# qc-tum/TNC

Measured on NVIDIA H100. Metric: pairwise contractions/sec (effective ZGEMM TFLOP/s in zgemm_tflops), higher is better.
Workload: dtype f64

## Files before the change

### include/tncb.h

```cpp
#ifndef TNCB_H
#define TNCB_H

#include <stddef.h>
#include <stdint.h>

#ifdef __cplusplus
extern "C" {
#endif

typedef enum tncb_status {
  TNCB_OK = 0,
  TNCB_ERR_INVALID = -1,
  TNCB_ERR_SHAPE = -2,
  TNCB_ERR_UNCONTRACTED = -3,
  TNCB_ERR_NOT_CONTRACTED = -4,
  TNCB_ERR_OOM = -5,
  TNCB_ERR_CUDA = -6,
  TNCB_ERR_GATE = -7,
  TNCB_ERR_NCCL = -8,
  TNCB_ERR_UNSUPPORTED = -9,
  TNCB_ERR_IO = -10
} tncb_status;

typedef struct tncb_ctx tncb_ctx;
// ... 8 lines not shown
int tncb_ctx_create(int device, size_t arena_bytes, tncb_ctx** out);
void tncb_ctx_destroy(tncb_ctx* ctx);
int tncb_ctx_synchronize(tncb_ctx* ctx);
void* tncb_ctx_stream(tncb_ctx* ctx);
int tncb_ctx_trim(tncb_ctx* ctx, uint64_t* freed_bytes, uint64_t* reserved_bytes);
int tncb_ctx_stats(tncb_ctx* ctx, uint64_t* kernel_launches, uint64_t* arena_peak_bytes,
                   uint64_t* arena_live_bytes);
int tncb_ctx_reset_stats(tncb_ctx* ctx);
int tncb_ctx_set_tcgen05_slices(tncb_ctx* ctx, int slices);
int tncb_ctx_set_tcgen05_engine(tncb_ctx* ctx, int engine);
int tncb_ctx_set_tolerance(tncb_ctx* ctx, double rel);
int tncb_ctx_set_tcgen05_moduli(tncb_ctx* ctx, int n_moduli);
int tncb_ctx_set_tcgen05_products(tncb_ctx* ctx, int products, long long min_k3);
int tncb_tcgen05_bound(uint64_t k, double rel, int n_moduli_force, int* n_moduli, int* bits_a, int* bits_b, double* bound);
int tncb_tcgen05_tables(int n_moduli, int* moduli, double* rho1, double* rho2, double* log2_product);
int tncb_ctx_set_tcgen05_workspace(tncb_ctx* ctx, size_t bytes);
int tncb_ctx_set_tcgen05_threshold(tncb_ctx* ctx, long long min_tiles, long long min_k);
int tncb_ctx_engine_counts(tncb_ctx* ctx, uint64_t counts[8]);
int tncb_ctx_last_tcgen05_info(tncb_ctx* ctx, double* int8_ops, int* n_moduli);
int tncb_ctx_last_tcgen05_products(tncb_ctx* ctx, int* products);
int tncb_ctx_time_gemm(tncb_ctx* ctx, int enable);
int tncb_ctx_last_gemm_ms(tncb_ctx* ctx, float* ms);
int tncb_ctx_gemm_totals(tncb_ctx* ctx, double* ms, double* int8_ops, uint64_t* launches);

int tncb_tensor_upload(tncb_ctx* ctx, int rank, const uint64_t* dims,
                       const double* host_re_im, tncb_tensor** out);
int tncb_tensor_alloc(tncb_ctx* ctx, int rank, const uint64_t* dims, tncb_tensor** out);
int tncb_tensor_download(tncb_ctx* ctx, const tncb_tensor* t, double* host_re_im);
int tncb_tensor_write(tncb_ctx* ctx, tncb_tensor* t, const double* host_re_im);
int tncb_tensor_read(tncb_ctx* ctx, const tncb_tensor* t, double* host_re_im);
int tncb_tensor_free(tncb_ctx* ctx, tncb_tensor* t);
int tncb_tensor_rank(const tncb_tensor* t);
int tncb_tensor_dims(const tncb_tensor* t, uint64_t* dims_out);
uint64_t tncb_tensor_elements(const tncb_tensor* t);
void* tncb_tensor_device_ptr(const tncb_tensor* t);

int tncb_contract_pair(tncb_ctx* ctx, int n_out, const uint64_t* out_legs,
                       int n_a, const uint64_t* a_legs, tncb_tensor* a,
                       int n_b, const uint64_t* b_legs, tncb_tensor* b,
                       tncb_tensor** out);
int tncb_contract_pair_keep(tncb_ctx* ctx, int n_a, const uint64_t* a_legs, const tncb_tensor* a,
                            int n_b, const uint64_t* b_legs, const tncb_tensor* b,
                            tncb_tensor** out);
int tncb_contract_pair_into(tncb_ctx* ctx, int n_a, const uint64_t* a_legs, const tncb_tensor* a,
                            int n_b, const uint64_t* b_legs, const tncb_tensor* b,
                            tncb_tensor* out);
// ... 137 lines not shown
```

### tnc_b200/__init__.py

```python
from __future__ import annotations

import ctypes as C
from typing import Sequence

import numpy as np

from ._lib import TncbError, check, lib, u64_array

__all__ = ["Context", "DeviceTensor", "TncbError", "contract_pair", "contract_pair_into", "default_context", "lib"]


class Context:

    def __init__(self, device: int = 0, arena_bytes: int = 0):
        self._l = lib()
        h = C.c_void_p()
        check(self._l.tncb_ctx_create(device, arena_bytes, C.byref(h)))
        self.handle = h
        self.device = device

    def synchronize(self) -> None:
        check(self._l.tncb_ctx_synchronize(self.handle))

    @property
# ... 31 lines not shown
    def engine_counts(self) -> dict:
        arr = (C.c_uint64 * 8)()
        check(self._l.tncb_ctx_engine_counts(self.handle, arr))
        names = ["k0", "k0_splitk", "k1_dmma", "k1_dmma_splitk", "k1_tcgen05", "k2", "permute", "reserved"]
        return {n: int(arr[i]) for i, n in enumerate(names)}

    def last_tcgen05_info(self) -> dict:
        ops, n = C.c_double(), C.c_int()
        check(self._l.tncb_ctx_last_tcgen05_info(self.handle, C.byref(ops), C.byref(n)))
        pr = C.c_int()
        check(self._l.tncb_ctx_last_tcgen05_products(self.handle, C.byref(pr)))
        return {"int8_ops": ops.value, "n_moduli": n.value, "products": pr.value}

    def set_tcgen05_threshold(self, min_tiles: int, min_k: int) -> None:
        check(self._l.tncb_ctx_set_tcgen05_threshold(self.handle, int(min_tiles), int(min_k)))

    def time_gemm(self, enable=True) -> None:
        check(self._l.tncb_ctx_time_gemm(self.handle, int(enable)))

    def gemm_totals(self) -> dict:
        ms, ops, n = C.c_double(), C.c_double(), C.c_uint64()
        check(self._l.tncb_ctx_gemm_totals(self.handle, C.byref(ms), C.byref(ops), C.byref(n)))
        return {"ms": ms.value, "int8_ops": ops.value, "launches": n.value}

    def last_gemm_ms(self) -> float:
        ms = C.c_float()
        check(self._l.tncb_ctx_last_gemm_ms(self.handle, C.byref(ms)))
        return float(ms.value)

    def reset_stats(self) -> None:
        check(self._l.tncb_ctx_reset_stats(self.handle))

    def close(self) -> None:
        if getattr(self, "handle", None):
            self._l.tncb_ctx_destroy(self.handle)
            self.handle = None

    def __del__(self):
        try:
            self.close()
        except Exception:
            pass


_default_ctx = None

# ... 161 lines not shown
```

### tnc_b200/_lib.py

```python
from __future__ import annotations

import ctypes as C
import os

_HERE = os.path.dirname(os.path.abspath(__file__))
LIB_PATH = os.path.join(_HERE, "lib", "libtncb200.so")

u64p = C.POINTER(C.c_uint64)
f64p = C.POINTER(C.c_double)
i32p = C.POINTER(C.c_int)
vpp = C.POINTER(C.c_void_p)


class TncbTn(C.Structure):
    pass


TncbTn._fields_ = [
    ("n_children", C.c_size_t),
    ("children", C.POINTER(TncbTn)),
    ("rank", C.c_int),
    ("legs", u64p),
    ("dims", u64p),
    ("kind", C.c_int),
# ... 27 lines not shown
    "tncb_ctx_create": (C.c_int, [C.c_int, C.c_size_t, vpp]),
    "tncb_ctx_destroy": (None, [C.c_void_p]),
    "tncb_ctx_synchronize": (C.c_int, [C.c_void_p]),
    "tncb_ctx_stream": (C.c_void_p, [C.c_void_p]),
    "tncb_ctx_stats": (C.c_int, [C.c_void_p, u64p, u64p, u64p]),
    "tncb_ctx_reset_stats": (C.c_int, [C.c_void_p]),
    "tncb_ctx_set_tcgen05_slices": (C.c_int, [C.c_void_p, C.c_int]),
    "tncb_ctx_set_tcgen05_engine": (C.c_int, [C.c_void_p, C.c_int]),
    "tncb_ctx_set_tolerance": (C.c_int, [C.c_void_p, C.c_double]),
    "tncb_ctx_set_tcgen05_moduli": (C.c_int, [C.c_void_p, C.c_int]),
    "tncb_tcgen05_bound": (C.c_int, [C.c_uint64, C.c_double, C.c_int, i32p, i32p, i32p, f64p]),
    "tncb_tcgen05_tables": (C.c_int, [C.c_int, i32p, f64p, f64p, f64p]),
    "tncb_ctx_set_tcgen05_workspace": (C.c_int, [C.c_void_p, C.c_size_t]),
    "tncb_ctx_engine_counts": (C.c_int, [C.c_void_p, u64p]),
    "tncb_ctx_last_tcgen05_info": (C.c_int, [C.c_void_p, f64p, i32p]),
    "tncb_ctx_last_tcgen05_products": (C.c_int, [C.c_void_p, i32p]),
    "tncb_ctx_trim": (C.c_int, [C.c_void_p, u64p, u64p]),
    "tncb_path_reconfigure": (C.c_int, [C.c_int, C.c_int, u64p, f64p, i32p, C.c_int, C.c_int, C.c_double, f64p, C.c_uint64, f64p, f64p, f64p]),
    "tncb_path_leg_scores": (C.c_int, [C.c_int, C.c_int, u64p, f64p, i32p, C.c_double, f64p, f64p, f64p, f64p, f64p]),
    "tncb_ctx_set_tcgen05_products": (C.c_int, [C.c_void_p, C.c_int, C.c_longlong]),
    "tncb_ctx_set_tcgen05_threshold": (C.c_int, [C.c_void_p, C.c_longlong, C.c_longlong]),
    "tncb_ctx_time_gemm": (C.c_int, [C.c_void_p, C.c_int]),
    "tncb_ctx_gemm_totals": (C.c_int, [C.c_void_p, f64p, f64p, u64p]),
    "tncb_ctx_last_gemm_ms": (C.c_int, [C.c_void_p, C.POINTER(C.c_float)]),
    "tncb_tensor_upload": (C.c_int, [C.c_void_p, C.c_int, u64p, C.c_void_p, vpp]),
    "tncb_tensor_alloc": (C.c_int, [C.c_void_p, C.c_int, u64p, vpp]),
    "tncb_tensor_download": (C.c_int, [C.c_void_p, C.c_void_p, C.c_void_p]),
    "tncb_tensor_write": (C.c_int, [C.c_void_p, C.c_void_p, C.c_void_p]),
    "tncb_tensor_read": (C.c_int, [C.c_void_p, C.c_void_p, C.c_void_p]),
    "tncb_tensor_free": (C.c_int, [C.c_void_p, C.c_void_p]),
    "tncb_tensor_rank": (C.c_int, [C.c_void_p]),
    "tncb_tensor_dims": (C.c_int, [C.c_void_p, u64p]),
    "tncb_tensor_elements": (C.c_uint64, [C.c_void_p]),
    "tncb_tensor_device_ptr": (C.c_void_p, [C.c_void_p]),
    "tncb_contract_pair": (C.c_int, [C.c_void_p, C.c_int, u64p, C.c_int, u64p, C.c_void_p, C.c_int, u64p, C.c_void_p, vpp]),
    "tncb_contract_pair_keep": (C.c_int, [C.c_void_p, C.c_int, u64p, C.c_void_p, C.c_int, u64p, C.c_void_p, vpp]),
    "tncb_contract_pair_into": (C.c_int, [C.c_void_p, C.c_int, u64p, C.c_void_p, C.c_int, u64p, C.c_void_p, C.c_void_p]),
    "tncb_contract_pair_host": (C.c_int, [C.c_void_p, C.c_int, u64p, u64p, C.c_void_p, C.c_int, u64p, u64p, C.c_void_p, C.c_void_p]),
    "tncb_pair_out_legs": (C.c_int, [C.c_int, u64p, u64p, C.c_int, u64p, u64p, i32p, u64p, u64p, u64p, u64p, u64p]),
    "tncb_pair_kernel_class": (C.c_int, [C.c_int, u64p, u64p, C.c_int, u64p, u64p]),
    "tncb_permute": (C.c_int, [C.c_void_p, C.c_void_p, i32p, vpp]),
    "tncb_conjugate": (C.c_int, [C.c_void_p, C.c_void_p]),
    "tncb_tensor_add": (C.c_int, [C.c_void_p, C.c_void_p, C.c_void_p]),
    "tncb_gate_matrix": (C.c_int, [C.c_char_p, f64p, C.c_int, C.c_int, f64p, i32p]),
    "tncb_contract_tensor_network": (C.c_int, [C.c_void_p, C.POINTER(TncbTn), C.POINTER(TncbPath), vpp, i32p, u64p]),
    "tncb_network_out_legs": (C.c_int, [C.POINTER(TncbTn), C.POINTER(TncbPath), i32p, u64p, u64p]),
# ... 90 lines not shown
```

### tnc_b200/csrc/crt.cu

```cuda
#include "internal.h"
#include "sm90.h"
#include <cuda.h>
#include <algorithm>
#include <cmath>
#include <cstdio>
#include <cstdlib>

namespace tncb {

constexpr int CRT_MAX_MOD = 20;
static const int kModuli[CRT_MAX_MOD] = {256, 253, 251, 249, 247, 245, 241, 239, 233, 229,
                                         227, 223, 211, 199, 197, 193, 191, 181, 179, 173};
constexpr int CRT_BT = 128;
constexpr int CRT_BKB = WG_BKB;
#ifndef CRT_RING3_STAGES
#define CRT_RING3_STAGES 3
#endif
#ifndef CRT_RING3_BK
#define CRT_RING3_BK 128
#endif
#ifndef CRT_RING4_STAGES
#define CRT_RING4_STAGES 5
#endif
#ifndef CRT_RING4_BK
// ... 126 lines not shown
#pragma unroll
  for (int it = 0; it < RES_ROWS_C * RES_K_C / 256; it++) {
    int r, k;
    crt_tile_coord(it * 256 + tid, lk, r, k);
    unsigned long long m = mv[it];
    for (int d = 1; d < (1 << lk); d <<= 1) m = max(m, __shfl_xor_sync(0xffffffffu, m, d));
    if (r != cur_r) {
      if (cur_m && (tid & ((1 << lk) - 1)) == 0) atomicMax(&s_max[cur_r], cur_m);
      cur_r = r; cur_m = 0ull;
    }
    cur_m = max(cur_m, m);
  }
  if (cur_m && (tid & ((1 << lk) - 1)) == 0) atomicMax(&s_max[cur_r], cur_m);
  __syncthreads();
  if (tid < RES_ROWS_C && row0 + tid < rows && s_max[tid] != 0ull) atomicMax(rowmax + row0 + tid, s_max[tid]);
}

__device__ __forceinline__ int crt_fix_byte(int s, int m) {
  if (s > 127) s -= m;
  else if (s < -128) s += m;
  return s;
}
constexpr int RES_ROWS = RES_ROWS_C, RES_K = RES_K_C, RES_RS = RES_K + RES_K / 8 + 1;
template <int COMPS, bool KARA>
__global__ void __launch_bounds__(256, 3)
crt_residue_kernel(const double2* __restrict__ src, const long long* __restrict__ off_row, const long long* __restrict__ off_k,
                   long long rows, long long K, long long rowsP, long long Kp, const unsigned long long* __restrict__ rowmax, int bits, int lk,
                   const __grid_constant__ CrtTables T, int8_t* __restrict__ planes) {
  extern __shared__ __align__(16) unsigned char res_smem_raw[];
  double2* tile = reinterpret_cast<double2*>(res_smem_raw);
  __shared__ double s_scale[RES_ROWS];
  __shared__ long long s_offr[RES_ROWS], s_offk[RES_K];
  __shared__ double s_inv[CRT_MAX_MOD];
  __shared__ int s_mod[CRT_MAX_MOD];
  const long long row0 = (long long)blockIdx.x * RES_ROWS, k0 = (long long)blockIdx.y * RES_K;
  const int tid = threadIdx.x;
  const double two_a = scalbn(1.0, bits);
  if (tid >= 64 && tid < 64 + CRT_MAX_MOD) { s_inv[tid - 64] = T.inv_mod[tid - 64]; s_mod[tid - 64] = T.mod[tid - 64]; }
  if (tid < RES_ROWS) {
    const long long r = row0 + tid;
    const int e = r < rows ? crt_exp_from_bits(rowmax[r]) : 0;
    s_scale[tid] = (e == kExpNonFinite) ? 0.0 : scalbn(1.0, -e);
    s_offr[tid] = r < rows ? __ldg(off_row + r) : -1;
  } else if (tid >= 128) {
    const int k = tid - 128;
    s_offk[k] = k0 + k < K ? __ldg(off_k + k0 + k) : -1;
  }
  __syncthreads();
  double2 vv[RES_ROWS * RES_K / 256];
#pragma unroll
  for (int it = 0; it < RES_ROWS * RES_K / 256; it++) {
    int r, k;
    crt_tile_coord(it * 256 + tid, lk, r, k);
    const long long orow = s_offr[r], ok = s_offk[k];
    vv[it] = make_double2(0.0, 0.0);
    if (orow >= 0 && ok >= 0) vv[it] = __ldg(src + orow + ok);
  }
#pragma unroll
  for (int it = 0; it < RES_ROWS * RES_K / 256; it++) {
    int r, k;
    crt_tile_coord(it * 256 + tid, lk, r, k);
    const double sc = s_scale[r];
    double2 v = vv[it];
    v.x = trunc(v.x * sc * two_a);
    v.y = trunc(v.y * sc * two_a);
    if (sc == 0.0) { v.x = 0.0; v.y = 0.0; }
    tile[r * RES_RS + k + (k >> 3)] = v;
  }
  __syncthreads();
  const int r = tid >> 3;
  if (row0 + r >= rows) return;
  const double RMAGIC = 6755399441055744.0;
  const long long plane_stride = rowsP * Kp;
#pragma unroll 1
  for (int pass = 0; pass < 2; pass++) {
    const int g = (tid & 7) + 8 * pass;
    double xr[8], xi[8];
    int lr[8], li[8];
#pragma unroll
    for (int j = 0; j < 8; j++) {
      const double2 v = tile[r * RES_RS + g * 9 + j];
      xr[j] = v.x; xi[j] = v.y;
      lr[j] = (int)__double2ll_rn(v.x); li[j] = (int)__double2ll_rn(v.y);
    }
    int8_t* dst = planes + (row0 + r) * Kp + k0 + g * 8;
    const int nmod = T.nmod;
#pragma unroll 1
    for (int i = 0; i < nmod; i++) {
      const int m = s_mod[i];
      const double inv = s_inv[i];
      uint32_t wr[2] = {0, 0}, wi[2] = {0, 0}, ws[2] = {0, 0};
#pragma unroll
      for (int j = 0; j < 8; j++) {
        const int qr = __double2loint(fma(xr[j], inv, RMAGIC));
        const int qi = __double2loint(fma(xi[j], inv, RMAGIC));
        const int rr = lr[j] - qr * m, ri = li[j] - qi * m;
        constexpr uint32_t sel[4] = {0x3214u, 0x3240u, 0x3410u, 0x4210u};
        wr[j >> 2] = __byte_perm(wr[j >> 2], (uint32_t)rr, sel[j & 3]);
        wi[j >> 2] = __byte_perm(wi[j >> 2], (uint32_t)ri, sel[j & 3]);
        if (KARA) ws[j >> 2] = __byte_perm(ws[j >> 2], (uint32_t)crt_fix_byte(rr + ri, m), sel[j & 3]);
      }
      int8_t* d = dst + (long long)i * (KARA ? 3 : COMPS) * plane_stride;
      if (KARA) {
        *reinterpret_cast<uint2*>(d) = make_uint2(wr[0], wr[1]);
        *reinterpret_cast<uint2*>(d + plane_stride) = make_uint2(wi[0], wi[1]);
        *reinterpret_cast<uint2*>(d + 2 * plane_stride) = make_uint2(ws[0], ws[1]);
      } else if (COMPS == 2) {
        *reinterpret_cast<uint2*>(d) = make_uint2(wr[0], wr[1]);
        *reinterpret_cast<uint2*>(d + plane_stride) = make_uint2(wi[0], wi[1]);
// ... 295 lines not shown
    return (size_t)nmod * (size_t)Kp * (size_t)(NPB * n_ + 3 * m_) + (size_t)nmod * nkc * NPR * (size_t)n_ * (size_t)m_;
  };
  while (ws_bytes(pn, pm) > budget && (pm > TM || pn > CRT_BT)) {
    if (pm >= pn && pm > TM) pm = round_up_ll(pm / 2, TM);
    else if (pn > CRT_BT) pn = round_up_ll(pn / 2, CRT_BT);
    else pm = round_up_ll(pm / 2, TM);
  }
  const size_t bytesB = (size_t)nmod * NPB * pn * Kp, bytesA = (size_t)nmod * 3 * pm * Kp;
  const size_t bytesR = (size_t)nmod * nkc * NPR * pn * pm;
  const size_t bytesE = (size_t)(pn + pm) * sizeof(unsigned long long);
  void *pb = nullptr, *pa = nullptr, *pr = nullptr, *pe = nullptr;
  int rc;
  if ((rc = ctx->arena.alloc(bytesB, &pb))) return rc;
  if ((rc = ctx->arena.alloc(bytesA, &pa))) { ctx->arena.free(pb, bytesB); return rc; }
  if ((rc = ctx->arena.alloc(bytesR, &pr))) { ctx->arena.free(pb, bytesB); ctx->arena.free(pa, bytesA); return rc; }
  if ((rc = ctx->arena.alloc(bytesE, &pe))) { ctx->arena.free(pb, bytesB); ctx->arena.free(pa, bytesA); ctx->arena.free(pr, bytesR); return rc; }
  auto cleanup = [&]() { ctx->arena.free(pb, bytesB); ctx->arena.free(pa, bytesA); ctx->arena.free(pr, bytesR); ctx->arena.free(pe, bytesE); };
  unsigned long long* max_n = (unsigned long long*)pe;
  unsigned long long* max_m = max_n + pn;

  static bool attr_done_dev[64] = {false};
  bool& attr_done = attr_done_dev[ctx->device & 63];
  const int smem_gemm4 = CrtRing<false>::SMEM, smem_gemm3 = CrtRing<true>::SMEM;
  const int smem_res = RES_ROWS * RES_RS * (int)sizeof(double2);
  if (!attr_done) {
    cudaError_t e = cudaFuncSetAttribute(crt_gemm_kernel<false>, cudaFuncAttributeMaxDynamicSharedMemorySize, smem_gemm4);
    if (e == cudaSuccess) e = cudaFuncSetAttribute(crt_gemm_kernel<true>, cudaFuncAttributeMaxDynamicSharedMemorySize, smem_gemm3);
    if (e == cudaSuccess) e = cudaFuncSetAttribute(crt_residue_kernel<2, false>, cudaFuncAttributeMaxDynamicSharedMemorySize, smem_res);
    if (e == cudaSuccess) e = cudaFuncSetAttribute(crt_residue_kernel<3, false>, cudaFuncAttributeMaxDynamicSharedMemorySize, smem_res);
    if (e == cudaSuccess) e = cudaFuncSetAttribute(crt_residue_kernel<2, true>, cudaFuncAttributeMaxDynamicSharedMemorySize, smem_res);
    if (e == cudaSuccess) e = cudaFuncSetAttribute(crt_residue_kernel<3, true>, cudaFuncAttributeMaxDynamicSharedMemorySize, smem_res);
    if (e != cudaSuccess) { cleanup(); return fail(TNCB_ERR_CUDA, cudaGetErrorString(e)); }
    attr_done = true;
  }
  auto lane_split = [](const LegList& kl, bool k_is_b, const LegList& fl) {
    auto p2 = [](long long d) { int b = 0; while ((2LL << b) <= d && b < 5) b++; return b; };
    const long long ks = kl.n ? (k_is_b ? kl.sb[kl.n - 1] : kl.sa[kl.n - 1]) : (1LL << 62);
    const long long fs = fl.n ? fl.sa[fl.n - 1] : (1LL << 62);
    if (ks <= fs) return kl.n ? p2(kl.dim[kl.n - 1]) : 0;
    return 0;
  };
  const int lk_b = lane_split(P.k, true, P.n), lk_a = lane_split(P.k, false, P.m);
  ctx->last_int8_ops = 0.0; ctx->last_nmod = nmod; ctx->last_products = kara ? 3 : 4;
  bool timed = false;

  for (long long n0 = 0; n0 < P.N; n0 += pn) {
    const long long nrows = std::min(pn, P.N - n0);
    const long long Np = round_up_ll(nrows, CRT_BT);
    if (Np != nrows) cudaMemsetAsync(pb, 0, (size_t)nmod * NPB * Np * Kp, st);
    cudaMemsetAsync(max_n, 0, (size_t)nrows * sizeof(unsigned long long), st);
    {
      dim3 g((unsigned)((nrows + RES_ROWS - 1) / RES_ROWS), (unsigned)(Kp / RES_K));
      crt_rowmax_kernel<<<g, 256, 0, st>>>(B, offBn + n0, offBk, nrows, P.K, lk_b, max_n);
      if (kara) crt_residue_kernel<2, true><<<g, 256, smem_res, st>>>(B, offBn + n0, offBk, nrows, P.K, Np, Kp, max_n, bits_b, lk_b, T, (int8_t*)pb);
      else crt_residue_kernel<2, false><<<g, 256, smem_res, st>>>(B, offBn + n0, offBk, nrows, P.K, Np, Kp, max_n, bits_b, lk_b, T, (int8_t*)pb);
    }
    ctx->launches += 2;
    CUtensorMap mapB;
    if ((rc = kara ? wg_make_map<CrtRing<true>::BK>(&mapB, pb, (uint64_t)nmod * NPB * Np, (uint64_t)Kp)
                   : wg_make_map<CrtRing<false>::BK>(&mapB, pb, (uint64_t)nmod * NPB * Np, (uint64_t)Kp))) { cleanup(); return rc; }
    for (long long m0 = 0; m0 < P.M; m0 += pm) {
      const long long mcols = std::min(pm, P.M - m0);
      const long long Mp = round_up_ll(mcols, TM);
      if (Mp != mcols) cudaMemsetAsync(pa, 0, (size_t)nmod * 3 * Mp * Kp, st);
      cudaMemsetAsync(max_m, 0, (size_t)mcols * sizeof(unsigned long long), st);
      {
        dim3 g((unsigned)((mcols + RES_ROWS - 1) / RES_ROWS), (unsigned)(Kp / RES_K));
        crt_rowmax_kernel<<<g, 256, 0, st>>>(A, offAm + m0, offAk, mcols, P.K, lk_a, max_m);
        if (kara) crt_residue_kernel<3, true><<<g, 256, smem_res, st>>>(A, offAm + m0, offAk, mcols, P.K, Mp, Kp, max_m, bits_a, lk_a, T, (int8_t*)pa);
        else crt_residue_kernel<3, false><<<g, 256, smem_res, st>>>(A, offAm + m0, offAk, mcols, P.K, Mp, Kp, max_m, bits_a, lk_a, T, (int8_t*)pa);
      }
      ctx->launches += 2;
      CUtensorMap mapA;
      if ((rc = kara ? wg_make_map<CrtRing<true>::BK>(&mapA, pa, (uint64_t)nmod * 3 * Mp, (uint64_t)Kp)
                     : wg_make_map<CrtRing<false>::BK>(&mapA, pa, (uint64_t)nmod * 3 * Mp, (uint64_t)Kp))) { cleanup(); return rc; }
      CrtGemmArgs g;
      g.R = (int8_t*)pr; g.Np = (int)Np; g.Mp = (int)Mp;
      g.tiles_n = (int)(Np / CRT_BT); g.tiles_m = (int)(Mp / TM); g.tile_m = TM;
      g.nmod = nmod; g.nkc = nkc; g.kb_per_chunk = kb_per_chunk; g.num_kb = num_kb;
      const long long items = (long long)g.tiles_n * g.tiles_m * nmod * nkc * (kara ? 3 : 1);
      if (items > 0x7fffffffLL) { cleanup(); return fail(TNCB_ERR_UNSUPPORTED, "too many work items"); }
      g.total_items = (int)items;
      g.group = ctx->crt_group;
      for (int i = 0; i < CRT_MAX_MOD; i++) { g.negmod[i] = -T.mod[i]; g.magic[i] = T.magic[i]; }
      const unsigned grid = (unsigned)std::min<long long>(ctas_max, items);
      const double ops = 2.0 * (kara ? 3.0 : 4.0) * (double)nmod * (double)Np * (double)Mp * (double)Kp;
      const bool time_this = ctx->time_gemm == 2 || (ctx->time_gemm == 1 && !timed);
      if (time_this) gemm_timer_begin(ctx);
      if (kara) crt_gemm_kernel<true><<<grid, WG_THREADS, smem_gemm3, st>>>(mapB, mapA, g);
      else crt_gemm_kernel<false><<<grid, WG_THREADS, smem_gemm4, st>>>(mapB, mapA, g);
      cudaError_t e = cudaGetLastError();
      if (time_this) { gemm_timer_end(ctx, ops); timed = true; }
      if (e != cudaSuccess) { cleanup(); return fail(TNCB_ERR_CUDA, std::string("crt_gemm_kernel launch: ") + cudaGetErrorString(e)); }
      ctx->last_int8_ops += ops;
      CrtReconArgs r;
      r.R = (const int8_t*)pr; r.C = C + n0 * P.M + m0; r.max_n = max_n; r.max_m = max_m;
      r.rows = nrows; r.cols = mcols; r.ldc = P.M; r.Np = Np; r.Mp = Mp; r.nkc = nkc;
      const long long threads = nrows * (Mp / 4);
      const unsigned rg = (unsigned)((threads + 255) / 256);
      if (kara) {
        if (nkc == 1) crt_reconstruct_kernel<true, true><<<rg, 256, 0, st>>>(r, T);
        else crt_reconstruct_kernel<false, true><<<rg, 256, 0, st>>>(r, T);
      } else {
        if (nkc == 1) crt_reconstruct_kernel<true, false><<<rg, 256, 0, st>>>(r, T);
        else crt_reconstruct_kernel<false, false><<<rg, 256, 0, st>>>(r, T);
      }
      ctx->launches += 2;
    }
  }
  ctx->engine_count[4]++;
  cudaError_t e = cudaGetLastError();
  cleanup();
  if (e != cudaSuccess) return fail(TNCB_ERR_CUDA, std::string("K1' (CRT) launch: ") + cudaGetErrorString(e));
  return TNCB_OK;
}

}
```

### tnc_b200/csrc/internal.h

```cpp
#pragma once
#include <cstdint>
#include <cstddef>
#include <string>
#include <vector>
#include <map>
#include <cuda_runtime.h>
#include "../../include/tncb.h"

namespace tncb {

constexpr int kMaxLegs = 64;
constexpr int kMaxGroups = 40;

struct LegList {
  int n;
  int _pad;
  long long dim[kMaxGroups];
  long long sa[kMaxGroups];
  long long sb[kMaxGroups];
};

struct PairPlan {
  std::vector<uint64_t> out_legs, out_dims;
  long long M = 1, N = 1, K = 1;
// ... 33 lines not shown
  uint64_t elems = 1;
  size_t bytes = 0;
  bool owned = true;
};

struct NcclApi;

struct tncb_ctx {
  int device = 0;
  cudaStream_t stream = nullptr;
  tncb::Arena arena;
  uint64_t launches = 0;
  int oz_slices = 8;
  int oz_engine = 0;
  long long oz_min_tiles = 96, oz_min_k = 1536;
  int crt_bits = 53; double crt_tol = 0.0; int crt_nmod_force = 0;
  long long crt_min_k = 256; double crt_min_mnk = 268435456.0;
  size_t crt_ws_bytes = (size_t)12 << 30; int crt_group = 8;
  double last_int8_ops = 0.0; int last_nmod = 0; int last_products = 0;
  int crt_products = 0;
  long long crt_kara_min_k = 2048;
  uint64_t engine_count[8] = {0, 0, 0, 0, 0, 0, 0, 0};
  int time_gemm = 0; cudaEvent_t gemm_ev0 = nullptr, gemm_ev1 = nullptr; bool gemm_ev_valid = false;
  std::vector<cudaEvent_t> gemm_pool; size_t gemm_used = 0; std::vector<double> gemm_ops;
  int sm_count = 132;
  void* stage_host = nullptr; size_t stage_bytes = 0;
  long long* tab = nullptr; size_t tab_elems = 0;
  bool tab_valid = false; tncb::LegList tab_m{}, tab_n{}, tab_k{};
  double2* partial = nullptr; size_t partial_elems = 0;
  double2* partial_override = nullptr; size_t partial_override_elems = 0;
  void* nccl_comm = nullptr; int world = 1, rank = 0;
  struct HostSlot { void* buf[3] = {nullptr, nullptr, nullptr}; size_t bytes[3] = {0, 0, 0};
                    cudaEvent_t in_done = nullptr, comp_done = nullptr, out_done = nullptr; bool busy = false; };
  HostSlot host_slot[3]; uint64_t host_jobs = 0;
  cudaStream_t h2d_stream = nullptr, d2h_stream = nullptr;
  std::vector<struct tncb_plan*> plans;
  struct CachedPlan { std::vector<uint64_t> key; struct tncb_plan* plan; };
  std::vector<CachedPlan> plan_cache;
};

extern "C" void tncb_plan_release_device_state(struct tncb_plan* plan);

namespace tncb {
int launch_pair(tncb_ctx* ctx, const PairPlan& p, const double2* A, const double2* B, double2* C,
                int count = 1, long long stride = 0);
int launch_permute(tncb_ctx* ctx, const double2* in, double2* out, int rank,
                   const uint64_t* in_dims, const int* perm);
int launch_conj(tncb_ctx* ctx, double2* data, uint64_t elems);
int launch_add(tncb_ctx* ctx, double2* dst, const double2* src, uint64_t elems);
int ensure_tab(tncb_ctx* ctx, size_t elems);
int launch_k1_ozaki(tncb_ctx* ctx, const PairPlan& p, const double2* A, const double2* B, double2* C, int S,
                    const long long* offAm, const long long* offBn, const long long* offAk, const long long* offBk);

int launch_k1_crt(tncb_ctx* ctx, const PairPlan& p, const double2* A, const double2* B, double2* C,
                  const long long* offAm, const long long* offBn, const long long* offAk, const long long* offBk);
void crt_choose(long long K, int want_bits, int nmod_force, int* nmod, int* bits_a, int* bits_b);
int crt_bits_for_tolerance(long long K, double tol);
int crt_export_tables(int nmod, int* moduli, double* rho1, double* rho2, double* log2_product);

void gemm_timer_begin(tncb_ctx* ctx);
void gemm_timer_end(tncb_ctx* ctx, double ops);

int ensure_partial(tncb_ctx* ctx, size_t elems);
size_t k0_partial_elems(int sm_count, const PairPlan& p);

constexpr int kBatchGroups = 8;
struct CompactLegs { int n; int _pad; long long dim[kBatchGroups]; long long sa[kBatchGroups]; long long sb[kBatchGroups]; };
struct K0BatchItem {
  long long offA, offB, offC;
  long long M, N, K;
  int G, _pad;
  CompactLegs m, n, k;
};
bool k0_batch_eligible(int sm_count, const PairPlan& p);
int k0_batch_fill(int sm_count, const PairPlan& p, K0BatchItem* item);
int launch_k0_batch(tncb_ctx* ctx, const K0BatchItem* d_items, const int* d_block_start, int n_items, int total_blocks, char* ws,
                    int count = 1, long long stride = 0);

constexpr int kGradGroups = 8;
struct GradItem {
  long long src;
  long long dst;
  long long elems;
  int n, _pad;
// ... 61 lines not shown
```

### tnc_b200/csrc/runtime.cu

```cuda
#include "internal.h"
#include <algorithm>
#include <cstdio>
#include <cstdlib>
#include <cstring>
#include <cmath>

namespace tncb {

static inline size_t round_up(size_t x, size_t a) { return (x + a - 1) / a * a; }

int Arena::alloc(size_t bytes, void** out) {
  bytes = round_up(std::max<size_t>(bytes, 256), 256);
  for (Slab& s : slabs) {
    for (auto it = s.free_by_off.begin(); it != s.free_by_off.end(); ++it) {
      if (it->second >= bytes) {
        size_t off = it->first, sz = it->second;
        s.free_by_off.erase(it);
        if (sz > bytes) s.free_by_off[off + bytes] = sz - bytes;
        *out = s.base + off;
        live += bytes; peak = std::max(peak, live);
        return TNCB_OK;
      }
    }
  }
// ... 40 lines not shown
    }
  }
}

void Arena::release_all() {
  for (Slab& s : slabs) cudaFree(s.base);
  slabs.clear(); reserved = live = 0;
}

size_t Arena::trim() {
  size_t freed = 0;
  for (size_t i = 0; i < slabs.size();) {
    Slab& s = slabs[i];
    if (s.free_by_off.size() == 1 && s.free_by_off.begin()->first == 0 && s.free_by_off.begin()->second == s.size) {
      cudaFree(s.base);
      freed += s.size; reserved -= s.size;
      slabs.erase(slabs.begin() + i);
    } else i++;
  }
  if (slabs.empty()) next_slab = (size_t)256 << 20;
  return freed;
}

void gemm_timer_begin(tncb_ctx* ctx) {
  if (ctx->time_gemm == 1) cudaEventRecord(ctx->gemm_ev0, ctx->stream);
  else if (ctx->time_gemm == 2) {
    if (ctx->gemm_used + 2 > ctx->gemm_pool.size()) {
      cudaEvent_t a, b; cudaEventCreate(&a); cudaEventCreate(&b);
      ctx->gemm_pool.push_back(a); ctx->gemm_pool.push_back(b);
    }
    cudaEventRecord(ctx->gemm_pool[ctx->gemm_used], ctx->stream);
  }
}

void gemm_timer_end(tncb_ctx* ctx, double ops) {
  if (ctx->time_gemm == 1) { cudaEventRecord(ctx->gemm_ev1, ctx->stream); ctx->gemm_ev_valid = true; }
  else if (ctx->time_gemm == 2) {
    cudaEventRecord(ctx->gemm_pool[ctx->gemm_used + 1], ctx->stream);
    ctx->gemm_used += 2; ctx->gemm_ops.push_back(ops);
  }
}

int tensor_new(tncb_ctx* ctx, int rank, const uint64_t* dims, tncb_tensor** out) {
  if (rank < 0 || rank > kMaxLegs) return fail(TNCB_ERR_INVALID, "tensor rank out of range");
  tncb_tensor* t = new tncb_tensor();
  t->rank = rank; t->elems = 1;
  for (int i = 0; i < rank; i++) { t->dims[i] = dims[i]; t->elems *= dims[i]; }
  t->bytes = std::max<size_t>(t->elems * sizeof(double2), 16);
  void* p = nullptr;
  int rc = ctx->arena.alloc(t->bytes, &p);
  if (rc) { delete t; return rc; }
  t->ptr = (double2*)p;
  *out = t;
  return TNCB_OK;
}

}

using namespace tncb;

extern "C" {

int tncb_ctx_create(int device, size_t arena_bytes, tncb_ctx** out) {
// ... 209 lines not shown
  if (!ctx || !counts) return fail(TNCB_ERR_INVALID, "null argument");
  for (int i = 0; i < 8; i++) counts[i] = ctx->engine_count[i];
  return TNCB_OK;
}

int tncb_ctx_last_tcgen05_info(tncb_ctx* ctx, double* int8_ops, int* n_moduli) {
  if (!ctx) return fail(TNCB_ERR_INVALID, "ctx is null");
  if (int8_ops) *int8_ops = ctx->last_int8_ops;
  if (n_moduli) *n_moduli = ctx->last_nmod;
  return TNCB_OK;
}

int tncb_ctx_set_tcgen05_threshold(tncb_ctx* ctx, long long min_tiles, long long min_k) {
  if (!ctx || min_tiles < 1 || min_k < 1) return fail(TNCB_ERR_INVALID, "bad argument");
  ctx->oz_min_tiles = min_tiles; ctx->oz_min_k = min_k;
  ctx->crt_min_k = min_k;
  ctx->crt_min_mnk = min_tiles <= 1 ? 0.0 : 268435456.0;
  return TNCB_OK;
}

int tncb_ctx_time_gemm(tncb_ctx* ctx, int enable) {
  if (!ctx) return fail(TNCB_ERR_INVALID, "ctx is null");
  TNCB_CUDA(cudaSetDevice(ctx->device));
  if (enable < 0 || enable > 2) return fail(TNCB_ERR_INVALID, "enable must be 0, 1 (last launch) or 2 (accumulate)");
  if (enable && !ctx->gemm_ev0) { TNCB_CUDA(cudaEventCreate(&ctx->gemm_ev0)); TNCB_CUDA(cudaEventCreate(&ctx->gemm_ev1)); }
  ctx->time_gemm = enable; ctx->gemm_ev_valid = false; ctx->gemm_used = 0; ctx->gemm_ops.clear();
  return TNCB_OK;
}

int tncb_ctx_gemm_totals(tncb_ctx* ctx, double* ms, double* ops, uint64_t* launches) {
  if (!ctx) return fail(TNCB_ERR_INVALID, "ctx is null");
  TNCB_CUDA(cudaSetDevice(ctx->device));
  TNCB_CUDA(cudaStreamSynchronize(ctx->stream));
  double tms = 0.0, tops = 0.0;
  for (size_t i = 0; i + 1 < ctx->gemm_used; i += 2) {
    float t = 0.f;
    TNCB_CUDA(cudaEventElapsedTime(&t, ctx->gemm_pool[i], ctx->gemm_pool[i + 1]));
    tms += t; tops += ctx->gemm_ops[i / 2];
  }
  if (ms) *ms = tms;
  if (ops) *ops = tops;
  if (launches) *launches = ctx->gemm_used / 2;
  ctx->gemm_used = 0; ctx->gemm_ops.clear();
  return TNCB_OK;
}

int tncb_ctx_last_gemm_ms(tncb_ctx* ctx, float* ms) {
  if (!ctx || !ms) return fail(TNCB_ERR_INVALID, "null argument");
  if (!ctx->gemm_ev_valid) return fail(TNCB_ERR_INVALID, "no timed GEMM kernel yet");
  TNCB_CUDA(cudaEventSynchronize(ctx->gemm_ev1));
  TNCB_CUDA(cudaEventElapsedTime(ms, ctx->gemm_ev0, ctx->gemm_ev1));
  return TNCB_OK;
}

int tncb_tensor_alloc(tncb_ctx* ctx, int rank, const uint64_t* dims, tncb_tensor** out) {
  if (!ctx || !out || (rank > 0 && !dims)) return fail(TNCB_ERR_INVALID, "null argument");
  TNCB_CUDA(cudaSetDevice(ctx->device));
  return tensor_new(ctx, rank, dims, out);
}

int tncb_tensor_upload(tncb_ctx* ctx, int rank, const uint64_t* dims, const double* host, tncb_tensor** out) {
  if (!host) return fail(TNCB_ERR_INVALID, "host buffer is null");
  int rc = tncb_tensor_alloc(ctx, rank, dims, out);
  if (rc) return rc;
  tncb_tensor* t = *out;
  TNCB_CUDA(cudaMemcpyAsync(t->ptr, host, t->elems * sizeof(double2), cudaMemcpyHostToDevice, ctx->stream));
// ... 130 lines not shown
```

Measured before the change: 5839.

## Double-buffer residue kernel with cp.async and multiple K tiles per CTA

The CRT residue kernel now runs 512 threads per CTA and loops over several K tiles per block. Each next tile is gathered into a second shared-memory buffer with cp.async while the current tile is reduced to int8 residue planes. The tiles-per-CTA count is chosen from grid size so there are still enough CTAs to fill the GPU. This targets load latency and per-CTA setup cost in the residue pass, at the price of twice the shared memory and lower occupancy (launch bounds 512,1). It also adds a per-pass timing mode and a pass_totals API for profiling.

```diff
diff --git a/include/tncb.h b/include/tncb.h
--- a/include/tncb.h
+++ b/include/tncb.h
@@ -54,6 +54,7 @@
 int tncb_ctx_time_gemm(tncb_ctx* ctx, int enable);
 int tncb_ctx_last_gemm_ms(tncb_ctx* ctx, float* ms);
 int tncb_ctx_gemm_totals(tncb_ctx* ctx, double* ms, double* int8_ops, uint64_t* launches);
+int tncb_ctx_pass_totals(tncb_ctx* ctx, double ms[4], uint64_t launches[4]);
 
 int tncb_tensor_upload(tncb_ctx* ctx, int rank, const uint64_t* dims,
                        const double* host_re_im, tncb_tensor** out);
diff --git a/tnc_b200/__init__.py b/tnc_b200/__init__.py
--- a/tnc_b200/__init__.py
+++ b/tnc_b200/__init__.py
@@ -77,6 +77,11 @@
         ms, ops, n = C.c_double(), C.c_double(), C.c_uint64()
         check(self._l.tncb_ctx_gemm_totals(self.handle, C.byref(ms), C.byref(ops), C.byref(n)))
         return {"ms": ms.value, "int8_ops": ops.value, "launches": n.value}
+
+    def pass_totals(self) -> dict:
+        ms, n = (C.c_double * 4)(), (C.c_uint64 * 4)()
+        check(self._l.tncb_ctx_pass_totals(self.handle, ms, n))
+        return {c: {"ms": ms[i], "launches": int(n[i])} for i, c in enumerate(("rowmax", "residue", "gemm", "reconstruct"))}
 
     def last_gemm_ms(self) -> float:
         ms = C.c_float()
diff --git a/tnc_b200/_lib.py b/tnc_b200/_lib.py
--- a/tnc_b200/_lib.py
+++ b/tnc_b200/_lib.py
@@ -73,6 +73,7 @@
     "tncb_ctx_set_tcgen05_threshold": (C.c_int, [C.c_void_p, C.c_longlong, C.c_longlong]),
     "tncb_ctx_time_gemm": (C.c_int, [C.c_void_p, C.c_int]),
     "tncb_ctx_gemm_totals": (C.c_int, [C.c_void_p, f64p, f64p, u64p]),
+    "tncb_ctx_pass_totals": (C.c_int, [C.c_void_p, f64p, u64p]),
     "tncb_ctx_last_gemm_ms": (C.c_int, [C.c_void_p, C.POINTER(C.c_float)]),
     "tncb_tensor_upload": (C.c_int, [C.c_void_p, C.c_int, u64p, C.c_void_p, vpp]),
     "tncb_tensor_alloc": (C.c_int, [C.c_void_p, C.c_int, u64p, vpp]),
diff --git a/tnc_b200/csrc/crt.cu b/tnc_b200/csrc/crt.cu
--- a/tnc_b200/csrc/crt.cu
+++ b/tnc_b200/csrc/crt.cu
@@ -172,18 +172,24 @@
   return s;
 }
 constexpr int RES_ROWS = RES_ROWS_C, RES_K = RES_K_C, RES_RS = RES_K + RES_K / 8 + 1;
+constexpr int RES_THREADS = 512, RES_TPC_MAX = 8;
+constexpr int RES_TILE = RES_ROWS * RES_RS;
+__device__ __forceinline__ void crt_cp_async16(void* dst, const void* src) {
+  asm volatile("cp.async.cg.shared.global [%0], [%1], 16;" :: "r"((uint32_t)__cvta_generic_to_shared(dst)), "l"(src) : "memory");
+}
 template <int COMPS, bool KARA>
-__global__ void __launch_bounds__(256, 3)
+__global__ void __launch_bounds__(RES_THREADS, 1)
 crt_residue_kernel(const double2* __restrict__ src, const long long* __restrict__ off_row, const long long* __restrict__ off_k,
                    long long rows, long long K, long long rowsP, long long Kp, const unsigned long long* __restrict__ rowmax, int bits, int lk,
-                   const __grid_constant__ CrtTables T, int8_t* __restrict__ planes) {
+                   int tpc, const __grid_constant__ CrtTables T, int8_t* __restrict__ planes) {
   extern __shared__ __align__(16) unsigned char res_smem_raw[];
-  double2* tile = reinterpret_cast<double2*>(res_smem_raw);
+  double2* tiles = reinterpret_cast<double2*>(res_smem_raw);
   __shared__ double s_scale[RES_ROWS];
-  __shared__ long long s_offr[RES_ROWS], s_offk[RES_K];
+  __shared__ long long s_offr[RES_ROWS], s_offk[RES_TPC_MAX * RES_K];
   __shared__ double s_inv[CRT_MAX_MOD];
   __shared__ int s_mod[CRT_MAX_MOD];
-  const long long row0 = (long long)blockIdx.x * RES_ROWS, k0 = (long long)blockIdx.y * RES_K;
+  const long long row0 = (long long)blockIdx.x * RES_ROWS, kbase = (long long)blockIdx.y * tpc * RES_K;
+  const int ntile = (int)min((long long)tpc, (Kp - kbase) / RES_K);
   const int tid = threadIdx.x;
   const double two_a = scalbn(1.0, bits);
   if (tid >= 64 && tid < 64 + CRT_MAX_MOD) { s_inv[tid - 64] = T.inv_mod[tid - 64]; s_mod[tid - 64] = T.mod[tid - 64]; }
@@ -192,39 +198,43 @@
     const int e = r < rows ? crt_exp_from_bits(rowmax[r]) : 0;
     s_scale[tid] = (e == kExpNonFinite) ? 0.0 : scalbn(1.0, -e);
     s_offr[tid] = r < rows ? __ldg(off_row + r) : -1;
-  } else if (tid >= 128) {
-    const int k = tid - 128;
-    s_offk[k] = k0 + k < K ? __ldg(off_k + k0 + k) : -1;
-  }
+  }
+  for (int k = tid; k < ntile * RES_K; k += RES_THREADS) s_offk[k] = kbase + k < K ? __ldg(off_k + kbase + k) : -1;
   __syncthreads();
-  double2 vv[RES_ROWS * RES_K / 256];
-#pragma unroll
-  for (int it = 0; it < RES_ROWS * RES_K / 256; it++) {
-    int r, k;
-    crt_tile_coord(it * 256 + tid, lk, r, k);
-    const long long orow = s_offr[r], ok = s_offk[k];
-    vv[it] = make_double2(0.0, 0.0);
-    if (orow >= 0 && ok >= 0) vv[it] = __ldg(src + orow + ok);
-  }
-#pragma unroll
-  for (int it = 0; it < RES_ROWS * RES_K / 256; it++) {
-    int r, k;
-    crt_tile_coord(it * 256 + tid, lk, r, k);
-    const double sc = s_scale[r];
-    double2 v = vv[it];
-    v.x = trunc(v.x * sc * two_a);
-    v.y = trunc(v.y * sc * two_a);
-    if (sc == 0.0) { v.x = 0.0; v.y = 0.0; }
-    tile[r * RES_RS + k + (k >> 3)] = v;
-  }
-  __syncthreads();
-  const int r = tid >> 3;
-  if (row0 + r >= rows) return;
+  auto gather = [&](int t) {
+    double2* tile = tiles + (t & 1) * RES_TILE;
+#pragma unroll
+    for (int it = 0; it < RES_ROWS * RES_K / RES_THREADS; it++) {
+      int r, k;
+      crt_tile_coord(it * RES_THREADS + tid, lk, r, k);
+      const long long orow = s_offr[r], ok = s_offk[t * RES_K + k];
+      double2* d = tile + r * RES_RS + k + (k >> 3);
+      if (orow >= 0 && ok >= 0) crt_cp_async16(d, src + orow + ok);
+      else *d = make_double2(0.0, 0.0);
+    }
+  };
+  gather(0);
+  const int r = tid >> 4, g = tid & 15;
   const double RMAGIC = 6755399441055744.0;
   const long long plane_stride = rowsP * Kp;
-#pragma unroll 1
-  for (int pass = 0; pass < 2; pass++) {
-    const int g = (tid & 7) + 8 * pass;
+  const int nmod = T.nmod;
+  for (int t = 0; t < ntile; t++) {
+    double2* tile = tiles + (t & 1) * RES_TILE;
+    asm volatile("cp.async.wait_all;" ::: "memory");
+#pragma unroll
+    for (int it = 0; it < RES_ROWS * RES_K / RES_THREADS; it++) {
+      int rr, k;
+      crt_tile_coord(it * RES_THREADS + tid, lk, rr, k);
+      const double sc = s_scale[rr];
+      double2 v = tile[rr * RES_RS + k + (k >> 3)];
+      v.x = trunc(v.x * sc * two_a);
+      v.y = trunc(v.y * sc * two_a);
+      if (sc == 0.0) { v.x = 0.0; v.y = 0.0; }
+      tile[rr * RES_RS + k + (k >> 3)] = v;
+    }
+    __syncthreads();
+    if (t + 1 < ntile) gather(t + 1);
+    if (row0 + r >= rows) continue;
     double xr[8], xi[8];
     int lr[8], li[8];
 #pragma unroll
@@ -233,8 +243,7 @@
       xr[j] = v.x; xi[j] = v.y;
       lr[j] = (int)__double2ll_rn(v.x); li[j] = (int)__double2ll_rn(v.y);
     }
-    int8_t* dst = planes + (row0 + r) * Kp + k0 + g * 8;
-    const int nmod = T.nmod;
+    int8_t* dst = planes + (row0 + r) * Kp + kbase + (long long)t * RES_K + g * 8;
 #pragma unroll 1
     for (int i = 0; i < nmod; i++) {
       const int m = s_mod[i];
@@ -576,7 +585,7 @@
   static bool attr_done_dev[64] = {false};
   bool& attr_done = attr_done_dev[ctx->device & 63];
   const int smem_gemm4 = CrtRing<false>::SMEM, smem_gemm3 = CrtRing<true>::SMEM;
-  const int smem_res = RES_ROWS * RES_RS * (int)sizeof(double2);
+  const int smem_res = 2 * RES_TILE * (int)sizeof(double2);
   if (!attr_done) {
     cudaError_t e = cudaFuncSetAttribute(crt_gemm_kernel<false>, cudaFuncAttributeMaxDynamicSharedMemorySize, smem_gemm4);
     if (e == cudaSuccess) e = cudaFuncSetAttribute(crt_gemm_kernel<true>, cudaFuncAttributeMaxDynamicSharedMemorySize, smem_gemm3);
@@ -595,8 +604,15 @@
     return 0;
   };
   const int lk_b = lane_split(P.k, true, P.n), lk_a = lane_split(P.k, false, P.m);
+  auto res_tiles_per_cta = [&](unsigned bands) {
+    const long long ktiles = Kp / RES_K;
+    int tpc = RES_TPC_MAX;
+    while (tpc > 1 && (long long)bands * ((ktiles + tpc - 1) / tpc) < 4LL * ctas_max) tpc >>= 1;
+    return (int)std::min<long long>(tpc, ktiles);
+  };
   ctx->last_int8_ops = 0.0; ctx->last_nmod = nmod; ctx->last_products = kara ? 3 : 4;
   bool timed = false;
+  const bool passes = ctx->time_gemm == 3;
 
   for (long long n0 = 0; n0 < P.N; n0 += pn) {
     const long long nrows = std::min(pn, P.N - n0);
@@ -604,10 +620,15 @@
     if (Np != nrows) cudaMemsetAsync(pb, 0, (size_t)nmod * NPB * Np * Kp, st);
     cudaMemsetAsync(max_n, 0, (size_t)nrows * sizeof(unsigned long long), st);
     {
-      dim3 g((unsigned)((nrows + RES_ROWS - 1) / RES_ROWS), (unsigned)(Kp / RES_K));
+      const unsigned bands = (unsigned)((nrows + RES_ROWS - 1) / RES_ROWS);
+      const int tpc = res_tiles_per_cta(bands);
+      dim3 g(bands, (unsigned)(Kp / RES_K)), gr(bands, (unsigned)((Kp / RES_K + tpc - 1) / tpc));
+      if (passes) pass_timer_begin(ctx);
       crt_rowmax_kernel<<<g, 256, 0, st>>>(B, offBn + n0, offBk, nrows, P.K, lk_b, max_n);
-      if (kara) crt_residue_kernel<2, true><<<g, 256, smem_res, st>>>(B, offBn + n0, offBk, nrows, P.K, Np, Kp, max_n, bits_b, lk_b, T, (int8_t*)pb);
-      else crt_residue_kernel<2, false><<<g, 256, smem_res, st>>>(B, offBn + n0, offBk, nrows, P.K, Np, Kp, max_n, bits_b, lk_b, T, (int8_t*)pb);
+      if (passes) { pass_timer_end(ctx, PASS_ROWMAX); pass_timer_begin(ctx); }
+      if (kara) crt_residue_kernel<2, true><<<gr, RES_THREADS, smem_res, st>>>(B, offBn + n0, offBk, nrows, P.K, Np, Kp, max_n, bits_b, lk_b, tpc, T, (int8_t*)pb);
+      else crt_residue_kernel<2, false><<<gr, RES_THREADS, smem_res, st>>>(B, offBn + n0, offBk, nrows, P.K, Np, Kp, max_n, bits_b, lk_b, tpc, T, (int8_t*)pb);
+      if (passes) pass_timer_end(ctx, PASS_RESIDUE);
     }
     ctx->launches += 2;
     CUtensorMap mapB;
@@ -619,10 +640,15 @@
       if (Mp != mcols) cudaMemsetAsync(pa, 0, (size_t)nmod * 3 * Mp * Kp, st);
       cudaMemsetAsync(max_m, 0, (size_t)mcols * sizeof(unsigned long long), st);
       {
-        dim3 g((unsigned)((mcols + RES_ROWS - 1) / RES_ROWS), (unsigned)(Kp / RES_K));
+        const unsigned bands = (unsigned)((mcols + RES_ROWS - 1) / RES_ROWS);
+        const int tpc = res_tiles_per_cta(bands);
+        dim3 g(bands, (unsigned)(Kp / RES_K)), gr(bands, (unsigned)((Kp / RES_K + tpc - 1) / tpc));
+        if (passes) pass_timer_begin(ctx);
         crt_rowmax_kernel<<<g, 256, 0, st>>>(A, offAm + m0, offAk, mcols, P.K, lk_a, max_m);
-        if (kara) crt_residue_kernel<3, true><<<g, 256, smem_res, st>>>(A, offAm + m0, offAk, mcols, P.K, Mp, Kp, max_m, bits_a, lk_a, T, (int8_t*)pa);
-        else crt_residue_kernel<3, false><<<g, 256, smem_res, st>>>(A, offAm + m0, offAk, mcols, P.K, Mp, Kp, max_m, bits_a, lk_a, T, (int8_t*)pa);
+        if (passes) { pass_timer_end(ctx, PASS_ROWMAX); pass_timer_begin(ctx); }
+        if (kara) crt_residue_kernel<3, true><<<gr, RES_THREADS, smem_res, st>>>(A, offAm + m0, offAk, mcols, P.K, Mp, Kp, max_m, bits_a, lk_a, tpc, T, (int8_t*)pa);
+        else crt_residue_kernel<3, false><<<gr, RES_THREADS, smem_res, st>>>(A, offAm + m0, offAk, mcols, P.K, Mp, Kp, max_m, bits_a, lk_a, tpc, T, (int8_t*)pa);
+        if (passes) pass_timer_end(ctx, PASS_RESIDUE);
       }
       ctx->launches += 2;
       CUtensorMap mapA;
@@ -639,7 +665,7 @@
       for (int i = 0; i < CRT_MAX_MOD; i++) { g.negmod[i] = -T.mod[i]; g.magic[i] = T.magic[i]; }
       const unsigned grid = (unsigned)std::min<long long>(ctas_max, items);
       const double ops = 2.0 * (kara ? 3.0 : 4.0) * (double)nmod * (double)Np * (double)Mp * (double)Kp;
-      const bool time_this = ctx->time_gemm == 2 || (ctx->time_gemm == 1 && !timed);
+      const bool time_this = ctx->time_gemm >= 2 || (ctx->time_gemm == 1 && !timed);
       if (time_this) gemm_timer_begin(ctx);
       if (kara) crt_gemm_kernel<true><<<grid, WG_THREADS, smem_gemm3, st>>>(mapB, mapA, g);
       else crt_gemm_kernel<false><<<grid, WG_THREADS, smem_gemm4, st>>>(mapB, mapA, g);
@@ -652,6 +678,7 @@
       r.rows = nrows; r.cols = mcols; r.ldc = P.M; r.Np = Np; r.Mp = Mp; r.nkc = nkc;
       const long long threads = nrows * (Mp / 4);
       const unsigned rg = (unsigned)((threads + 255) / 256);
+      if (passes) pass_timer_begin(ctx);
       if (kara) {
         if (nkc == 1) crt_reconstruct_kernel<true, true><<<rg, 256, 0, st>>>(r, T);
         else crt_reconstruct_kernel<false, true><<<rg, 256, 0, st>>>(r, T);
@@ -659,6 +686,7 @@
         if (nkc == 1) crt_reconstruct_kernel<true, false><<<rg, 256, 0, st>>>(r, T);
         else crt_reconstruct_kernel<false, false><<<rg, 256, 0, st>>>(r, T);
       }
+      if (passes) pass_timer_end(ctx, PASS_RECONSTRUCT);
       ctx->launches += 2;
     }
   }
diff --git a/tnc_b200/csrc/internal.h b/tnc_b200/csrc/internal.h
--- a/tnc_b200/csrc/internal.h
+++ b/tnc_b200/csrc/internal.h
@@ -79,7 +79,7 @@
   long long crt_kara_min_k = 2048;
   uint64_t engine_count[8] = {0, 0, 0, 0, 0, 0, 0, 0};
   int time_gemm = 0; cudaEvent_t gemm_ev0 = nullptr, gemm_ev1 = nullptr; bool gemm_ev_valid = false;
-  std::vector<cudaEvent_t> gemm_pool; size_t gemm_used = 0; std::vector<double> gemm_ops;
+  std::vector<cudaEvent_t> gemm_pool; size_t gemm_used = 0; std::vector<double> gemm_ops; std::vector<int> gemm_cls;
   int sm_count = 132;
   void* stage_host = nullptr; size_t stage_bytes = 0;
   long long* tab = nullptr; size_t tab_elems = 0;
@@ -117,6 +117,9 @@
 
 void gemm_timer_begin(tncb_ctx* ctx);
 void gemm_timer_end(tncb_ctx* ctx, double ops);
+enum { PASS_ROWMAX = 0, PASS_RESIDUE = 1, PASS_GEMM = 2, PASS_RECONSTRUCT = 3, PASS_CLASSES = 4 };
+void pass_timer_begin(tncb_ctx* ctx);
+void pass_timer_end(tncb_ctx* ctx, int cls, double ops = 0.0);
 
 int ensure_partial(tncb_ctx* ctx, size_t elems);
 size_t k0_partial_elems(int sm_count, const PairPlan& p);
diff --git a/tnc_b200/csrc/runtime.cu b/tnc_b200/csrc/runtime.cu
--- a/tnc_b200/csrc/runtime.cu
+++ b/tnc_b200/csrc/runtime.cu
@@ -86,23 +86,27 @@
   return freed;
 }
 
+void pass_timer_begin(tncb_ctx* ctx) {
+  if (ctx->gemm_used + 2 > ctx->gemm_pool.size()) {
+    cudaEvent_t a, b; cudaEventCreate(&a); cudaEventCreate(&b);
+    ctx->gemm_pool.push_back(a); ctx->gemm_pool.push_back(b);
+  }
+  cudaEventRecord(ctx->gemm_pool[ctx->gemm_used], ctx->stream);
+}
+
+void pass_timer_end(tncb_ctx* ctx, int cls, double ops) {
+  cudaEventRecord(ctx->gemm_pool[ctx->gemm_used + 1], ctx->stream);
+  ctx->gemm_used += 2; ctx->gemm_ops.push_back(ops); ctx->gemm_cls.push_back(cls);
+}
+
 void gemm_timer_begin(tncb_ctx* ctx) {
   if (ctx->time_gemm == 1) cudaEventRecord(ctx->gemm_ev0, ctx->stream);
-  else if (ctx->time_gemm == 2) {
-    if (ctx->gemm_used + 2 > ctx->gemm_pool.size()) {
-      cudaEvent_t a, b; cudaEventCreate(&a); cudaEventCreate(&b);
-      ctx->gemm_pool.push_back(a); ctx->gemm_pool.push_back(b);
-    }
-    cudaEventRecord(ctx->gemm_pool[ctx->gemm_used], ctx->stream);
-  }
+  else if (ctx->time_gemm >= 2) pass_timer_begin(ctx);
 }
 
 void gemm_timer_end(tncb_ctx* ctx, double ops) {
   if (ctx->time_gemm == 1) { cudaEventRecord(ctx->gemm_ev1, ctx->stream); ctx->gemm_ev_valid = true; }
-  else if (ctx->time_gemm == 2) {
-    cudaEventRecord(ctx->gemm_pool[ctx->gemm_used + 1], ctx->stream);
-    ctx->gemm_used += 2; ctx->gemm_ops.push_back(ops);
-  }
+  else if (ctx->time_gemm >= 2) pass_timer_end(ctx, PASS_GEMM, ops);
 }
 
 int tensor_new(tncb_ctx* ctx, int rank, const uint64_t* dims, tncb_tensor** out) {
@@ -358,26 +362,42 @@
 int tncb_ctx_time_gemm(tncb_ctx* ctx, int enable) {
   if (!ctx) return fail(TNCB_ERR_INVALID, "ctx is null");
   TNCB_CUDA(cudaSetDevice(ctx->device));
-  if (enable < 0 || enable > 2) return fail(TNCB_ERR_INVALID, "enable must be 0, 1 (last launch) or 2 (accumulate)");
+  if (enable < 0 || enable > 3) return fail(TNCB_ERR_INVALID, "enable must be 0, 1 (last launch), 2 (accumulate) or 3 (accumulate per pass)");
   if (enable && !ctx->gemm_ev0) { TNCB_CUDA(cudaEventCreate(&ctx->gemm_ev0)); TNCB_CUDA(cudaEventCreate(&ctx->gemm_ev1)); }
-  ctx->time_gemm = enable; ctx->gemm_ev_valid = false; ctx->gemm_used = 0; ctx->gemm_ops.clear();
-  return TNCB_OK;
-}
-
-int tncb_ctx_gemm_totals(tncb_ctx* ctx, double* ms, double* ops, uint64_t* launches) {
-  if (!ctx) return fail(TNCB_ERR_INVALID, "ctx is null");
+  ctx->time_gemm = enable; ctx->gemm_ev_valid = false; ctx->gemm_used = 0; ctx->gemm_ops.clear(); ctx->gemm_cls.clear();
+  return TNCB_OK;
+}
+
+int tncb_ctx_pass_totals(tncb_ctx* ctx, double ms[4], uint64_t launches[4]) {
+  if (!ctx || !ms || !launches) return fail(TNCB_ERR_INVALID, "null argument");
   TNCB_CUDA(cudaSetDevice(ctx->device));
   TNCB_CUDA(cudaStreamSynchronize(ctx->stream));
-  double tms = 0.0, tops = 0.0;
+  for (int c = 0; c < PASS_CLASSES; c++) { ms[c] = 0.0; launches[c] = 0; }
   for (size_t i = 0; i + 1 < ctx->gemm_used; i += 2) {
     float t = 0.f;
     TNCB_CUDA(cudaEventElapsedTime(&t, ctx->gemm_pool[i], ctx->gemm_pool[i + 1]));
-    tms += t; tops += ctx->gemm_ops[i / 2];
+    ms[ctx->gemm_cls[i / 2]] += t; launches[ctx->gemm_cls[i / 2]]++;
+  }
+  ctx->gemm_used = 0; ctx->gemm_ops.clear(); ctx->gemm_cls.clear();
+  return TNCB_OK;
+}
+
+int tncb_ctx_gemm_totals(tncb_ctx* ctx, double* ms, double* ops, uint64_t* launches) {
+  if (!ctx) return fail(TNCB_ERR_INVALID, "ctx is null");
+  TNCB_CUDA(cudaSetDevice(ctx->device));
+  TNCB_CUDA(cudaStreamSynchronize(ctx->stream));
+  double tms = 0.0, tops = 0.0;
+  uint64_t n = 0;
+  for (size_t i = 0; i + 1 < ctx->gemm_used; i += 2) {
+    if (ctx->gemm_cls[i / 2] != PASS_GEMM) continue;
+    float t = 0.f;
+    TNCB_CUDA(cudaEventElapsedTime(&t, ctx->gemm_pool[i], ctx->gemm_pool[i + 1]));
+    tms += t; tops += ctx->gemm_ops[i / 2]; n++;
   }
   if (ms) *ms = tms;
   if (ops) *ops = tops;
-  if (launches) *launches = ctx->gemm_used / 2;
-  ctx->gemm_used = 0; ctx->gemm_ops.clear();
+  if (launches) *launches = n;
+  ctx->gemm_used = 0; ctx->gemm_ops.clear(); ctx->gemm_cls.clear();
   return TNCB_OK;
 }
 
```

Measured after the change: 5981, median of 6. +2.4%, better.
